# mtumalan/VisionTransformer

Measured on AMD Instinct MI355X. Metric: images/sec (512×512) ViT-B/16 seg, 1/2/4/8 MI355X + mask argmax match, higher is better.
Workload: dtype f32

## Files before the change

visiontransformer_amd/csrc/attention_bf16.hip:

```cpp
#include <type_traits>

#include "kernels.hpp"

namespace vitseg {
namespace {

constexpr int HD = 64;
constexpr int QB = 128;
constexpr int KB = 64;
constexpr float LOG2E = 1.4426950408889634f;
typedef short s16x4 __attribute__((ext_vector_type(4)));
typedef float f32x2 __attribute__((ext_vector_type(2)));

__device__ __forceinline__ int kappa(int s, int h) { return (s & 3) + 8 * (s >> 2) + 4 * h; }

template <bool DROP, bool RAGGED, bool MW, typename H>
__global__ __launch_bounds__(256, 3) void attn_bf16_kernel(const bf16_t* __restrict__ qkv, bf16_t* __restrict__ ctx,
                                                           float* __restrict__ lse, int B, int Np, int A,
                                                           DropArgs dr, const unsigned* __restrict__ maskw) {
    static_assert(!MW || (DROP && !RAGGED), "mask words: dropout on, whole 128-query blocks");
    __shared__ __attribute__((aligned(16))) bf16_t lds[2][2][KB * HD];

    const int tid = threadIdx.x, lane = tid & 63, wave = tid >> 6;
    const int li = lane & 31, lh = lane >> 5;
    const AttnTile at = attn_tile((Np + QB - 1) / QB, A);
    const int head = at.head, b = at.b;
    const int D = A * HD, ld = 3 * D;
    const size_t row0 = (size_t)b * Np;
    const size_t cls_row = (size_t)B * Np + b;
    const bf16_t* qbase = qkv + head * HD;
    const bf16_t* kbase = qkv + D + head * HD;
    const bf16_t* vbase = qkv + 2 * D + head * HD;
    const float c = 0.125f * LOG2E;

    const int q_local = at.rt * QB + wave * 32 + li;
    const bool q_valid = !RAGGED || q_local < Np;
    const size_t q_row = row0 + (q_valid ? q_local : Np - 1);
    f32x4 qf[4];
#pragma unroll
    for (int s = 0; s < 4; ++s) qf[s] = *(const f32x4*)(qbase + q_row * ld + 16 * s + 8 * lh);

    const unsigned dkey = drop_key(dr.seed, dr.stream, (unsigned)((b * A + head) * (Np + 1) + q_local));
    float m_run, l_run;
    f32x16 o[2];
    {
        float part = 0.f;
#pragma unroll
        for (int s = 0; s < 4; ++s) {
            const f32x4 kc = *(const f32x4*)(kbase + cls_row * ld + 16 * s + 8 * lh);
#pragma unroll
            for (int e = 0; e < 4; ++e) {
                const unsigned qu = __float_as_uint(qf[s][e]), ku = __float_as_uint(kc[e]);
                part = fmaf(H16<H>::lo(qu), H16<H>::lo(ku), part);
                part = fmaf(H16<H>::hi(qu), H16<H>::hi(ku), part);
            }
        }
        m_run = part + __shfl_xor(part, 32, 64);
        l_run = lh == 0 ? 1.f : 0.f;
// ... 21 lines not shown
    {
        const unsigned long long base = (unsigned long long)(kbase + row0 * ld);
        kv_rsrc[0] = (int)(unsigned)base;
        kv_rsrc[1] = (int)(unsigned)((base >> 32) & 0xffffu);
        kv_rsrc[2] = Np * ld * 2;
        kv_rsrc[3] = 0x00020000;
    }
    const int drow = 16 * __builtin_amdgcn_readfirstlane(wave) + (lane >> 3);
    unsigned voff_k[2], voff_v[2];
#pragma unroll
    for (int pc = 0; pc < 2; ++pc) {
        const int key = drow + 8 * pc;
        voff_k[pc] = (unsigned)(key * ld * 2 + (((lane & 7) ^ ((key >> 1) & 7)) << 4));
        voff_v[pc] = (unsigned)(key * ld * 2 + D * 2 + (((lane & 7) ^ (((key >> 1) & 1) << 2)) << 4));
    }
    const unsigned lds_base = (unsigned)(size_t)(__attribute__((address_space(3))) char*)&lds[0][0][0];
    auto stage = [&](int kt, int buf) {
        const unsigned soff = (unsigned)(kt * KB * ld * 2);
        const unsigned dst = lds_base + (unsigned)(buf * 2 * KB * HD * 2) + (unsigned)(__builtin_amdgcn_readfirstlane(wave) * 2048);
#pragma unroll
        for (int pc = 0; pc < 2; ++pc) {
            asm volatile("s_mov_b32 m0, %0\n\ts_nop 0\n\tbuffer_load_dwordx4 %1, %2, %3 offen lds"
                         :: "s"(dst + pc * 1024), "v"(voff_k[pc]), "s"(kv_rsrc), "s"(soff) : "memory");
            asm volatile("s_mov_b32 m0, %0\n\ts_nop 0\n\tbuffer_load_dwordx4 %1, %2, %3 offen lds"
                         :: "s"(dst + KB * HD * 2 + pc * 1024), "v"(voff_v[pc]), "s"(kv_rsrc), "s"(soff) : "memory");
        }
    };
    const int k_off = li * HD;
    const int k_sw = (li >> 1) & 7;
    const int g = lane & 15, grp = lane >> 4, tq = g >> 2, tp = g & 3;
    const int v_row = 4 * (grp >> 1) + tq;
    const int v_sw = ((tq >> 1) & 1) << 2;
    const int v_dchunk = 2 * (grp & 1) + (tp >> 1), v_half = (tp & 1) * 4;

    const int nkt = (Np + KB - 1) / KB;
    const unsigned long* mrow = nullptr;
    if (MW) {
        const int nb = Np >> 5, qg = at.rt * 4 + __builtin_amdgcn_readfirstlane(wave);
        mrow = (const unsigned long*)maskw + ((size_t)((b * A + head) * nb + qg) * nb) * 16;
    }
    TileMasks lm;
    if (MW) lm.load(mrow);
    stage(0, 0);
    asm volatile("s_waitcnt vmcnt(0)" ::: "memory");
    __syncthreads();
    constexpr float PSUM_LIMIT = sizeof(H) == 2 && std::is_same<H, f16_t>::value ? 4096.f : 65536.f;
    for (int kt = 0; kt < nkt; ++kt) {
        const int buf = kt & 1;
        if (MW) lm.wait();
        const bf16_t* Ks = lds[buf][0];
        const bf16_t* Vs = lds[buf][1];

        f32x16 st[2];
        auto scores = [&]() {
#pragma unroll
            for (int kb = 0; kb < 2; ++kb) {
#pragma unroll
                for (int r = 0; r < 16; ++r) st[kb][r] = 0.f;
#pragma unroll
                for (int s = 0; s < 4; ++s) {
                    const f32x4 kf = *(const f32x4*)&Ks[kb * 32 * HD + k_off + (((2 * s + lh) ^ k_sw) << 3)];
                    st[kb] = H16<H>::mfma(__builtin_bit_cast(bf16x8, kf), __builtin_bit_cast(bf16x8, qf[s]), st[kb]);
                }
            }
            if (RAGGED) {
#pragma unroll
                for (int kb = 0; kb < 2; ++kb)
#pragma unroll
                    for (int r = 0; r < 16; ++r)
                        if (kt * KB + kb * 32 + kappa(r, lh) >= Np) st[kb][r] = -INFINITY;
            }
        };
        scores();
        stage(min(kt + 1, nkt - 1), buf ^ 1);
        float nmc = -m_run * c;
        float psum;
        unsigned pk[2][8];
        auto exponentiate = [&]() {
            float ps0 = 0.f, ps1 = 0.f;
#pragma unroll
            for (int kb = 0; kb < 2; ++kb)
#pragma unroll
                for (int r = 0; r < 16; r += 2) {
                    float p0 = __builtin_amdgcn_exp2f(fmaf(st[kb][r], c, nmc));
                    float p1 = __builtin_amdgcn_exp2f(fmaf(st[kb][r + 1], c, nmc));
                    ps0 += p0;
                    ps1 += p1;
                    if (MW) {
                        p0 = mask_select(lm.reg(kb, r), p0);
                        p1 = mask_select(lm.reg(kb, r + 1), p1);
                    } else if (DROP) {
                        const unsigned k0 = (unsigned)(kt * KB + kb * 32);
                        p0 = drop_keep(dkey, k0 + kappa(r, lh), dr.thresh) ? p0 * dr.scale : 0.f;
                        p1 = drop_keep(dkey, k0 + kappa(r + 1, lh), dr.thresh) ? p1 * dr.scale : 0.f;
                    }
                    pk[kb][r >> 1] = H16<H>::pack2(p0, p1);
                    asm volatile("" : "+v"(pk[kb][r >> 1]));
                }
            psum = ps0 + ps1;
        };
        exponentiate();
        if (__builtin_amdgcn_ballot_w64(!(psum <= PSUM_LIMIT)) != 0) {
            scores();
            float mx = fmaxf(st[0][0], st[1][0]);
#pragma unroll
            for (int r = 1; r < 16; r += 1) mx = fmaxf(fmaxf(mx, st[0][r]), st[1][r]);
            mx = fmaxf(mx, __shfl_xor(mx, 32, 64));
            const float delta = fmaxf(mx - m_run, 0.f);
            const float alpha = __builtin_amdgcn_exp2f(-delta * c);
            l_run *= alpha;
#pragma unroll
            for (int dt = 0; dt < 2; ++dt)
#pragma unroll
                for (int r = 0; r < 16; ++r) o[dt][r] *= alpha;
            m_run += delta;
            nmc = -m_run * c;
            exponentiate();
        }
        l_run += psum;

#pragma unroll
        for (int kb = 0; kb < 2; ++kb)
#pragma unroll
            for (int s = 0; s < 2; ++s) {
                const bf16x8 pf = __builtin_bit_cast(
                    bf16x8, (uint4){pk[kb][4 * s], pk[kb][4 * s + 1], pk[kb][4 * s + 2], pk[kb][4 * s + 3]});
#pragma unroll
                for (int dt = 0; dt < 2; ++dt) {
                    const int row_a = kb * 32 + 16 * s + v_row;
                    const int ch = (4 * dt + v_dchunk) ^ v_sw;
                    const s16x4 lo = __builtin_amdgcn_ds_read_tr16_b64_v4i16(
                        (__attribute__((address_space(3))) s16x4*)(Vs + row_a * HD + (ch << 3) + v_half));
                    const s16x4 hi = __builtin_amdgcn_ds_read_tr16_b64_v4i16(
                        (__attribute__((address_space(3))) s16x4*)(Vs + (row_a + 8) * HD + (ch << 3) + v_half));
                    const bf16x8 vf = {lo[0], lo[1], lo[2], lo[3], hi[0], hi[1], hi[2], hi[3]};
                    o[dt] = H16<H>::mfma(vf, pf, o[dt]);
                }
            }

        if (MW) lm.load(mrow + (size_t)min(kt + 1, nkt - 1) * 32);
        asm volatile("s_waitcnt vmcnt(0)" ::: "memory");
        __syncthreads();
    }
    if (MW) lm.wait();

    const float l_tot = l_run + __shfl_xor(l_run, 32, 64);
    const float inv = (MW ? dr.scale : 1.0f) / l_tot;
    if (lse && q_valid && lh == 0)
        lse[((size_t)b * A + head) * (Np + 1) + q_local] = m_run * c + __builtin_amdgcn_logf(l_tot);
    if (q_valid) {
        bf16_t* out = ctx + q_row * (size_t)D + head * HD;
#pragma unroll
        for (int dt = 0; dt < 2; ++dt)
#pragma unroll
            for (int g4 = 0; g4 < 4; ++g4) {
                uint2 t;
                t.x = H16<H>::pack2(o[dt][4 * g4] * inv, o[dt][4 * g4 + 1] * inv);
                t.y = H16<H>::pack2(o[dt][4 * g4 + 2] * inv, o[dt][4 * g4 + 3] * inv);
                *(uint2*)(out + dt * 32 + 8 * g4 + 4 * lh) = t;
            }
    }
}

template <typename H>
__global__ __launch_bounds__(1024) void attn_cls_bf16_kernel(const bf16_t* __restrict__ qkv, bf16_t* __restrict__ ctx,
                                                            float* __restrict__ lse, int B, int Np, int A,
                                                            DropArgs dr) {
    extern __shared__ __attribute__((aligned(16))) float sm[];
    const int N = Np + 1;
    float* sc = sm;
    float* red = sm + ((N + 63) & ~63);
    const int tid = threadIdx.x, lane = tid & 63, wave = tid >> 6;
    const int head = blockIdx.x, b = blockIdx.y;
    const int D = A * HD, ld = 3 * D;
    const size_t row0 = (size_t)b * Np, cls_row = (size_t)B * Np + b;
    const bf16_t* qp = qkv + cls_row * ld + head * HD;
    const bf16_t* kbase = qkv + D + head * HD;
    const bf16_t* vbase = qkv + 2 * D + head * HD;
    const int sub = lane & 15, grp = lane >> 4;

    const uint2 qu = *(const uint2*)(qp + 4 * sub);
    const float qs = 0.125f * LOG2E;
    const float q0 = H16<H>::lo(qu.x) * qs, q1 = H16<H>::hi(qu.x) * qs, q2 = H16<H>::lo(qu.y) * qs, q3 = H16<H>::hi(qu.y) * qs;
    for (int base = wave * 4; base < N; base += 256) {
        float part[4];
#pragma unroll
        for (int u = 0; u < 4; ++u) {
            const int key = base + 64 * u + grp;
            part[u] = 0.f;
            if (key < N) {
                const size_t row = key < Np ? row0 + key : cls_row;
                const uint2 ku = *(const uint2*)(kbase + row * ld + 4 * sub);
                part[u] = q0 * H16<H>::lo(ku.x) + q1 * H16<H>::hi(ku.x) + q2 * H16<H>::lo(ku.y) + q3 * H16<H>::hi(ku.y);
            }
        }
#pragma unroll
        for (int u = 0; u < 4; ++u) {
            float pu = part[u];
            pu = row16_sum(pu);
            const int key = base + 64 * u + grp;
            if (sub == 0 && key < N) sc[key] = pu;
        }
    }
    __syncthreads();
    float mx = -INFINITY;
    for (int i = tid; i < N; i += 1024) mx = fmaxf(mx, sc[i]);
    mx = wave_max(mx);
    if (lane == 0) red[wave] = mx;
    __syncthreads();
    mx = red[0];
    for (int w = 1; w < 16; ++w) mx = fmaxf(mx, red[w]);
    __syncthreads();
    float sum = 0.f;
    for (int i = tid; i < N; i += 1024) {
        const float pv = __builtin_amdgcn_exp2f(sc[i] - mx);
        sc[i] = pv;
        sum += pv;
    }
    sum = wave_sum(sum);
    if (lane == 0) red[wave] = sum;
    __syncthreads();
    float ltot = 0.f;
    for (int w = 0; w < 16; ++w) ltot += red[w];
    const float inv = 1.0f / ltot;
    if (lse && tid == 0) lse[((size_t)b * A + head) * N + Np] = mx + __builtin_amdgcn_logf(ltot);
    __syncthreads();
    const int kg = tid >> 4;
    f32x4 acc = {0.f, 0.f, 0.f, 0.f};
    for (int key0 = kg; key0 < N; key0 += 256) {
        uint2 vu[4];
        float pv[4];
#pragma unroll
        for (int u = 0; u < 4; ++u) {
            const int key = min(key0 + 64 * u, N - 1);
            const size_t row = key < Np ? row0 + key : cls_row;
            vu[u] = *(const uint2*)(vbase + row * ld + 4 * sub);
            pv[u] = key0 + 64 * u < N ? sc[key] : 0.f;
            if (dr.thresh)
                pv[u] = drop_keep(drop_key(dr.seed, dr.stream, (unsigned)((b * A + head) * N + Np)), (unsigned)key,
                                  dr.thresh) ? pv[u] * dr.scale : 0.f;
        }
#pragma unroll
        for (int u = 0; u < 4; ++u) {
            acc[0] = fmaf(pv[u], H16<H>::lo(vu[u].x), acc[0]);
            acc[1] = fmaf(pv[u], H16<H>::hi(vu[u].x), acc[1]);
            acc[2] = fmaf(pv[u], H16<H>::lo(vu[u].y), acc[2]);
            acc[3] = fmaf(pv[u], H16<H>::hi(vu[u].y), acc[3]);
        }
    }
    *(f32x4*)&red[kg * 64 + 4 * sub] = acc;
    __syncthreads();
    if (tid < 64) {
        float s = 0.f;
        for (int gI = 0; gI < 64; ++gI) s += red[gI * 64 + tid];
        ctx[cls_row * (size_t)D + head * HD + tid] = H16<H>::bits(s * inv);
    }
}

}

template <typename H>
static int launch_attention_h16(const void* qkv, void* ctx, float* lse, int B, int Np, int A, DropArgs dr, hipStream_t s,
                                const unsigned* maskw) {
    VITSEG_CHECK_ARG(qkv && ctx && B > 0 && Np > 0 && A > 0, VITSEG_EINVAL, "attention_bf16: bad arguments");
    const dim3 grid((unsigned)((Np + QB - 1) / QB) * A * B);
    const bool ragged = Np % QB != 0, drop = dr.thresh != 0;
#define VITSEG_ATTN_LAUNCH(DR, RG, MWORDS)                                                                           \
    hipLaunchKernelGGL((attn_bf16_kernel<DR, RG, MWORDS, H>), grid, dim3(256), 0, s, (const bf16_t*)qkv, (bf16_t*)ctx, \
                       lse, B, Np, A, dr, maskw)
    if (drop) {
        if (ragged) VITSEG_ATTN_LAUNCH(true, true, false);
        else if (maskw) VITSEG_ATTN_LAUNCH(true, false, true);
        else VITSEG_ATTN_LAUNCH(true, false, false);
    } else {
        if (ragged) VITSEG_ATTN_LAUNCH(false, true, false); else VITSEG_ATTN_LAUNCH(false, false, false);
    }
#undef VITSEG_ATTN_LAUNCH
    VITSEG_LAUNCH_CHECK("attn_bf16");
    const size_t smem = (size_t)(((Np + 1 + 63) & ~63) + 64 * 64) * sizeof(float);
    VITSEG_CHECK_ARG(smem <= 64 * 1024, VITSEG_ESHAPE, "attention_bf16: sequence too long for the CLS kernel");
    hipLaunchKernelGGL(attn_cls_bf16_kernel<H>, dim3(A, B), dim3(1024), smem, s, (const bf16_t*)qkv, (bf16_t*)ctx, lse, B,
                       Np, A, dr);
    VITSEG_LAUNCH_CHECK("attn_cls_bf16");
    return VITSEG_OK;
}

int launch_attention_bf16(const void* qkv, void* ctx, float* lse, int B, int Np, int A, DropArgs dr, hipStream_t s,
                          bool f16, const unsigned* maskw) {
    return f16 ? launch_attention_h16<f16_t>(qkv, ctx, lse, B, Np, A, dr, s, maskw)
               : launch_attention_h16<bf16_t>(qkv, ctx, lse, B, Np, A, dr, s, maskw);
}

}
```

visiontransformer_amd/csrc/attention_f32.hip:

```cpp
#include "kernels.hpp"

namespace vitseg {
namespace {

constexpr int HD = 64;
constexpr int QB = 128;
constexpr int KB = 64;
constexpr float LOG2E = 1.4426950408889634f;

__device__ __forceinline__ int kappa(int s, int h) { return (s & 3) + 8 * (s >> 2) + 4 * h; }

template <bool RAGGED>
__global__ __launch_bounds__(256, 2) void attn_f32_kernel(const float* __restrict__ qkv, float* __restrict__ ctx,
                                                          float* __restrict__ lse, int B, int Np, int A,
                                                          DropArgs dr) {
    __shared__ __attribute__((aligned(16))) float lds[2][2][KB * HD];

    const int tid = threadIdx.x, lane = tid & 63, wave = tid >> 6;
    const int li = lane & 31, lh = lane >> 5;
    const AttnTile at = attn_tile((Np + QB - 1) / QB, A);
    const int head = at.head, b = at.b;
    const int D = A * HD, ld = 3 * D;
    const size_t row0 = (size_t)b * Np;
    const size_t cls_row = (size_t)B * Np + b;
// ... 245 lines not shown
#pragma unroll
            for (int g4 = 0; g4 < 4; ++g4) {
                f32x4 t;
#pragma unroll
                for (int e = 0; e < 4; ++e) t[e] = o[dt][4 * g4 + e] * inv;
                *(f32x4*)(out + dt * 32 + 8 * g4 + 4 * lh) = t;
            }
    }
    if (cls_blk) {
        float* red = &lds[0][0][0];
        *(f32x4*)&red[cks * 64 + 4 * cq] = co;
        if (cq == 0) {
            red[1024 + cks] = cm;
            red[1040 + cks] = cl;
        }
        __syncthreads();
        if (tid < 64) {
            float M = red[1024];
#pragma unroll
            for (int g = 1; g < 16; ++g) M = fmaxf(M, red[1024 + g]);
            float L = 0.f, O = 0.f;
#pragma unroll
            for (int g = 0; g < 16; ++g) {
                const float w = __builtin_amdgcn_exp2f(red[1024 + g] - M);
                L = fmaf(red[1040 + g], w, L);
                O = fmaf(red[g * 64 + tid], w, O);
            }
            ctx[cls_row * (size_t)D + head * HD + tid] = O / L;
            if (lse && tid == 0) lse[((size_t)b * A + head) * (Np + 1) + Np] = M + __builtin_amdgcn_logf(L);
        }
    }
}

__global__ __launch_bounds__(1024) void attn_cls_f32_kernel(const float* __restrict__ qkv, float* __restrict__ ctx,
                                                           float* __restrict__ lse, int B, int Np, int A,
                                                           DropArgs dr) {
    extern __shared__ __attribute__((aligned(16))) float sm[];
    const int N = Np + 1;
    float* sc = sm;
    float* red = sm + ((N + 63) & ~63);
    const int tid = threadIdx.x, lane = tid & 63, wave = tid >> 6;
    const int head = blockIdx.x, b = blockIdx.y;
    const int D = A * HD, ld = 3 * D;
    const size_t row0 = (size_t)b * Np, cls_row = (size_t)B * Np + b;
    const float* qp = qkv + cls_row * ld + head * HD;
    const float* kbase = qkv + D + head * HD;
    const float* vbase = qkv + 2 * D + head * HD;
    const int sub = lane & 15, grp = lane >> 4;

    f32x4 q4 = *(const f32x4*)(qp + 4 * sub);
    const float qs = 0.125f * LOG2E;
    for (int e = 0; e < 4; ++e) q4[e] *= qs;
    for (int base = wave * 4; base < N; base += 256) {
        float part[4];
#pragma unroll
        for (int u = 0; u < 4; ++u) {
            const int key = base + 64 * u + grp;
            part[u] = 0.f;
            if (key < N) {
                const size_t row = key < Np ? row0 + key : cls_row;
                const f32x4 k4 = *(const f32x4*)(kbase + row * ld + 4 * sub);
                part[u] = q4[0] * k4[0] + q4[1] * k4[1] + q4[2] * k4[2] + q4[3] * k4[3];
            }
        }
#pragma unroll
        for (int u = 0; u < 4; ++u) {
            float pu = part[u];
            pu = row16_sum(pu);
            const int key = base + 64 * u + grp;
            if (sub == 0 && key < N) sc[key] = pu;
        }
    }
    __syncthreads();
    float mx = -INFINITY;
    for (int i = tid; i < N; i += 1024) mx = fmaxf(mx, sc[i]);
    mx = wave_max(mx);
    if (lane == 0) red[wave] = mx;
    __syncthreads();
    mx = red[0];
    for (int w = 1; w < 16; ++w) mx = fmaxf(mx, red[w]);
    __syncthreads();
    float sum = 0.f;
    for (int i = tid; i < N; i += 1024) {
        const float pv = __builtin_amdgcn_exp2f(sc[i] - mx);
        sc[i] = pv;
        sum += pv;
    }
    sum = wave_sum(sum);
    if (lane == 0) red[wave] = sum;
    __syncthreads();
    float ltot = 0.f;
    for (int w = 0; w < 16; ++w) ltot += red[w];
    const float inv = 1.0f / ltot;
    if (lse && tid == 0) lse[((size_t)b * A + head) * N + Np] = mx + __builtin_amdgcn_logf(ltot);
    __syncthreads();
    const int kg = tid >> 4;
    f32x4 acc = {0.f, 0.f, 0.f, 0.f};
    for (int key0 = kg; key0 < N; key0 += 256) {
        f32x4 v4[4];
        float pv[4];
#pragma unroll
        for (int u = 0; u < 4; ++u) {
            const int key = min(key0 + 64 * u, N - 1);
            const size_t row = key < Np ? row0 + key : cls_row;
            v4[u] = *(const f32x4*)(vbase + row * ld + 4 * sub);
            pv[u] = key0 + 64 * u < N ? sc[key] : 0.f;
            if (dr.thresh)
                pv[u] = drop_keep(drop_key(dr.seed, dr.stream, (unsigned)((b * A + head) * N + Np)), (unsigned)key,
                                  dr.thresh) ? pv[u] * dr.scale : 0.f;
        }
#pragma unroll
        for (int u = 0; u < 4; ++u)
            for (int e = 0; e < 4; ++e) acc[e] = fmaf(pv[u], v4[u][e], acc[e]);
    }
    *(f32x4*)&red[kg * 64 + 4 * sub] = acc;
    __syncthreads();
    if (tid < 64) {
        float s = 0.f;
        for (int g = 0; g < 64; ++g) s += red[g * 64 + tid];
        ctx[cls_row * (size_t)D + head * HD + tid] = s * inv;
    }
}

}

int launch_attention_f32(const float* qkv, float* ctx, float* lse, int B, int Np, int A, DropArgs dr, hipStream_t s,
                         bool x3) {
    VITSEG_CHECK_ARG(qkv && ctx && B > 0 && Np > 0 && A > 0, VITSEG_EINVAL, "attention_f32: bad arguments");
    const dim3 grid((unsigned)((Np + QB - 1) / QB) * A * B);
    if (x3) {
        VITSEG_CHECK_ARG(!lse && !dr.thresh, VITSEG_EINVAL, "attention (x3) is an inference path: no lse / dropout");
        if (int rc = launch_attention_x3_main(qkv, ctx, B, Np, A, s)) return rc;
    } else if (Np % QB == 0) {
        hipLaunchKernelGGL(attn_f32_kernel<false>, grid, dim3(256), 0, s, qkv, ctx, lse, B, Np, A, dr);
    } else {
        hipLaunchKernelGGL(attn_f32_kernel<true>, grid, dim3(256), 0, s, qkv, ctx, lse, B, Np, A, dr);
    }
    VITSEG_LAUNCH_CHECK("attn_f32");
    if (!x3) return VITSEG_OK;
    const size_t smem = (size_t)(((Np + 1 + 63) & ~63) + 64 * 64) * sizeof(float);
    VITSEG_CHECK_ARG(smem <= 64 * 1024, VITSEG_ESHAPE, "attention_f32: sequence too long for the CLS kernel");
    hipLaunchKernelGGL(attn_cls_f32_kernel, dim3(A, B), dim3(1024), smem, s, qkv, ctx, lse, B, Np, A, dr);
    VITSEG_LAUNCH_CHECK("attn_cls_f32");
    return VITSEG_OK;
}

}
```

visiontransformer_amd/csrc/attention_x3.hip:

```cpp
#include "kernels.hpp"

namespace vitseg {
namespace {

constexpr int HD = 64;
constexpr int QB = 128;
constexpr int KB = 64;
constexpr float LOG2E = 1.4426950408889634f;
constexpr float LO_SCALE = 2048.f, LO_INV = 1.0f / 2048.f;
typedef short s16x4 __attribute__((ext_vector_type(4)));

__device__ __forceinline__ int kappa(int s, int h) { return (s & 3) + 8 * (s >> 2) + 4 * h; }

__device__ __forceinline__ void split8(const f32x4& a, const f32x4& b, f32x4& hi, f32x4& lo) {
    unsigned h[4], l[4];
#pragma unroll
    for (int j = 0; j < 2; ++j) {
        const _Float16 a0 = (_Float16)a[2 * j], a1 = (_Float16)a[2 * j + 1];
        const _Float16 b0 = (_Float16)b[2 * j], b1 = (_Float16)b[2 * j + 1];
        h[j] = __builtin_bit_cast(unsigned, f16x2{a0, a1});
        h[2 + j] = __builtin_bit_cast(unsigned, f16x2{b0, b1});
        l[j] = H16<f16_t>::pack2((a[2 * j] - (float)a0) * LO_SCALE, (a[2 * j + 1] - (float)a1) * LO_SCALE);
        l[2 + j] = H16<f16_t>::pack2((b[2 * j] - (float)b0) * LO_SCALE, (b[2 * j + 1] - (float)b1) * LO_SCALE);
    }
    hi = __builtin_bit_cast(f32x4, (uint4){h[0], h[1], h[2], h[3]});
    lo = __builtin_bit_cast(f32x4, (uint4){l[0], l[1], l[2], l[3]});
}

template <bool RAGGED>
__global__ __launch_bounds__(256, 2) void attn_x3_kernel(const float* __restrict__ qkv, float* __restrict__ ctx, int B, int Np,
                                                         int A) {
    __shared__ __attribute__((aligned(16))) unsigned short lds[2][2][2][KB * HD];

    const int tid = threadIdx.x, lane = tid & 63, wave = tid >> 6;
    const int li = lane & 31, lh = lane >> 5;
    const AttnTile at = attn_tile((Np + QB - 1) / QB, A);
    const int head = at.head, b = at.b;
    const int D = A * HD, ld = 3 * D;
    const size_t row0 = (size_t)b * Np;
    const size_t cls_row = (size_t)B * Np + b;
    const float* qbase = qkv + head * HD;
    const float* kbase = qkv + D + head * HD;
    const float* vbase = qkv + 2 * D + head * HD;
    const float c = 0.125f * LOG2E;

    const int q_local = at.rt * QB + wave * 32 + li;
    const bool q_valid = q_local < Np;
    const size_t q_row = row0 + (q_valid ? q_local : Np - 1);
    f32x4 qh[4], ql[4];
    float m_run, l_run;
    f32x16 o0[2], o1[2];
    {
        float part = 0.f;
#pragma unroll
        for (int s = 0; s < 4; ++s) {
            const float* qp = qbase + q_row * ld + 16 * s + 8 * lh;
            const float* kp = kbase + cls_row * ld + 16 * s + 8 * lh;
            const f32x4 qa = *(const f32x4*)qp, qb = *(const f32x4*)(qp + 4);
            const f32x4 ka = *(const f32x4*)kp, kb = *(const f32x4*)(kp + 4);
#pragma unroll
            for (int e = 0; e < 4; ++e) part = fmaf(qb[e], kb[e], fmaf(qa[e], ka[e], part));
            split8(qa, qb, qh[s], ql[s]);
        }
        m_run = part + __shfl_xor(part, 32, 64);
        l_run = lh == 0 ? 1.f : 0.f;
#pragma unroll
        for (int dt = 0; dt < 2; ++dt)
#pragma unroll
            for (int g4 = 0; g4 < 4; ++g4) {
// ... 11 lines not shown
    auto gload = [&](int kt) {
#pragma unroll
        for (int i = 0; i < 2; ++i) {
            int key = kt * KB + lr + 32 * i;
            if (RAGGED) key = min(key, Np - 1);
            const size_t off = (row0 + key) * ld + 8 * lc;
            rk[i][0] = *(const f32x4*)(kbase + off);
            rk[i][1] = *(const f32x4*)(kbase + off + 4);
            rv[i][0] = *(const f32x4*)(vbase + off);
            rv[i][1] = *(const f32x4*)(vbase + off + 4);
        }
    };
    auto swrite = [&](int buf) {
#pragma unroll
        for (int i = 0; i < 2; ++i) {
            const int key = lr + 32 * i;
            f32x4 hi, lo;
            split8(rk[i][0], rk[i][1], hi, lo);
            const int kpos = key * HD + ((lc ^ ((key >> 1) & 7)) << 3);
            *(f32x4*)&lds[buf][0][0][kpos] = hi;
            *(f32x4*)&lds[buf][0][1][kpos] = lo;
            split8(rv[i][0], rv[i][1], hi, lo);
            const int vpos = key * HD + ((lc ^ (((key >> 1) & 1) << 2)) << 3);
            *(f32x4*)&lds[buf][1][0][vpos] = hi;
            *(f32x4*)&lds[buf][1][1][vpos] = lo;
        }
    };
    const int k_off = li * HD;
    const int k_sw = (li >> 1) & 7;
    const int g = lane & 15, grp = lane >> 4, tq = g >> 2, tp = g & 3;
    const int v_row = 4 * (grp >> 1) + tq;
    const int v_sw = ((tq >> 1) & 1) << 2;
    const int v_dchunk = 2 * (grp & 1) + (tp >> 1), v_half = (tp & 1) * 4;

    const int nkt = (Np + KB - 1) / KB;
    gload(0);
    swrite(0);
    __syncthreads();
    for (int kt = 0; kt < nkt; ++kt) {
        const int buf = kt & 1;
        gload(min(kt + 1, nkt - 1));
        __builtin_amdgcn_sched_barrier(0);
        const unsigned short* Kh = lds[buf][0][0];
        const unsigned short* Kl = lds[buf][0][1];
        const unsigned short* Vh = lds[buf][1][0];
        const unsigned short* Vl = lds[buf][1][1];

        f32x16 st[2];
#pragma unroll
        for (int kb = 0; kb < 2; ++kb) {
            f32x16 s1;
#pragma unroll
            for (int r = 0; r < 16; ++r) st[kb][r] = s1[r] = 0.f;
#pragma unroll
            for (int s = 0; s < 4; ++s) {
                const int pos = kb * 32 * HD + k_off + (((2 * s + lh) ^ k_sw) << 3);
                const bf16x8 kh = __builtin_bit_cast(bf16x8, *(const f32x4*)&Kh[pos]);
                const bf16x8 kl = __builtin_bit_cast(bf16x8, *(const f32x4*)&Kl[pos]);
                st[kb] = H16<f16_t>::mfma(kh, __builtin_bit_cast(bf16x8, qh[s]), st[kb]);
                s1 = H16<f16_t>::mfma(kl, __builtin_bit_cast(bf16x8, qh[s]), s1);
                s1 = H16<f16_t>::mfma(kh, __builtin_bit_cast(bf16x8, ql[s]), s1);
            }
#pragma unroll
            for (int r = 0; r < 16; ++r) st[kb][r] = fmaf(s1[r], LO_INV, st[kb][r]);
        }
        if (RAGGED) {
#pragma unroll
            for (int kb = 0; kb < 2; ++kb)
#pragma unroll
                for (int r = 0; r < 16; ++r)
                    if (kt * KB + kb * 32 + kappa(r, lh) >= Np) st[kb][r] = -INFINITY;
        }
        float mx = fmaxf(st[0][0], st[1][0]);
#pragma unroll
        for (int r = 1; r < 16; r += 1) mx = fmaxf(fmaxf(mx, st[0][r]), st[1][r]);
        mx = fmaxf(mx, __shfl_xor(mx, 32, 64));
        const float m_new = fmaxf(m_run, mx);
        if (__builtin_amdgcn_ballot_w64(m_new > m_run) != 0) {
            const float alpha = __builtin_amdgcn_exp2f((m_run - m_new) * c);
// ... 36 lines not shown
                    const int row_a = kb * 32 + 16 * s + v_row;
                    const int ch = (4 * dt + v_dchunk) ^ v_sw;
                    const int p0 = row_a * HD + (ch << 3) + v_half, p8 = (row_a + 8) * HD + (ch << 3) + v_half;
                    const s16x4 hlo = __builtin_amdgcn_ds_read_tr16_b64_v4i16((__attribute__((address_space(3))) s16x4*)(Vh + p0));
                    const s16x4 hhi = __builtin_amdgcn_ds_read_tr16_b64_v4i16((__attribute__((address_space(3))) s16x4*)(Vh + p8));
                    const s16x4 llo = __builtin_amdgcn_ds_read_tr16_b64_v4i16((__attribute__((address_space(3))) s16x4*)(Vl + p0));
                    const s16x4 lhi = __builtin_amdgcn_ds_read_tr16_b64_v4i16((__attribute__((address_space(3))) s16x4*)(Vl + p8));
                    const bf16x8 vh = {hlo[0], hlo[1], hlo[2], hlo[3], hhi[0], hhi[1], hhi[2], hhi[3]};
                    const bf16x8 vl = {llo[0], llo[1], llo[2], llo[3], lhi[0], lhi[1], lhi[2], lhi[3]};
                    o0[dt] = H16<f16_t>::mfma(vh, pfh, o0[dt]);
                    o1[dt] = H16<f16_t>::mfma(vl, pfh, o1[dt]);
                    o1[dt] = H16<f16_t>::mfma(vh, pfl, o1[dt]);
                }
            }

        swrite(buf ^ 1);
        __syncthreads();
    }

    const float l_tot = l_run + __shfl_xor(l_run, 32, 64);
    const float inv = 1.0f / l_tot;
    if (q_valid) {
        float* out = ctx + q_row * (size_t)D + head * HD;
#pragma unroll
        for (int dt = 0; dt < 2; ++dt)
#pragma unroll
            for (int g4 = 0; g4 < 4; ++g4) {
                f32x4 t;
#pragma unroll
                for (int e = 0; e < 4; ++e) t[e] = fmaf(o1[dt][4 * g4 + e], LO_INV, o0[dt][4 * g4 + e]) * inv;
                *(f32x4*)(out + dt * 32 + 8 * g4 + 4 * lh) = t;
            }
    }
}

}

int launch_attention_x3_main(const float* qkv, float* ctx, int B, int Np, int A, hipStream_t s) {
    const dim3 grid((unsigned)((Np + QB - 1) / QB) * A * B);
    if (Np % QB == 0)
        hipLaunchKernelGGL(attn_x3_kernel<false>, grid, dim3(256), 0, s, qkv, ctx, B, Np, A);
    else
        hipLaunchKernelGGL(attn_x3_kernel<true>, grid, dim3(256), 0, s, qkv, ctx, B, Np, A);
    VITSEG_LAUNCH_CHECK("attn_x3");
    return VITSEG_OK;
}

}
```

visiontransformer_amd/csrc/common.hpp:

```cpp
#pragma once
#include <hip/hip_runtime.h>
#include <stdint.h>

#include "../../include/vitseg.h"

namespace vitseg {

constexpr int WAVE = 64;

typedef float f32x4 __attribute__((ext_vector_type(4)));
typedef float f32x16 __attribute__((ext_vector_type(16)));
typedef short bf16x8 __attribute__((ext_vector_type(8)));
typedef short bf16x4 __attribute__((ext_vector_type(4)));

void set_error(const char* fmt, ...);
int hip_fail(hipError_t e, const char* what);

enum Opt {
    OPT_NO_F32P = 0,
    OPT_NO_P8,
    OPT_NO_H16P,
    OPT_NO_RAGGED_P8,
    OPT_NO_DROPMASK,
    OPT_DROPW_LIMIT_MB,
// ... 15 lines not shown
        if (!(cond)) {                    \
            ::vitseg::set_error(__VA_ARGS__); \
            return (code);                \
        }                                 \
    } while (0)

#define VITSEG_LAUNCH_CHECK(what)                               \
    do {                                                        \
        hipError_t e__ = hipGetLastError();                     \
        if (e__ != hipSuccess) return ::vitseg::hip_fail(e__, what); \
    } while (0)

inline size_t up256(size_t v) { return (v + 255) & ~(size_t)255; }

__device__ __forceinline__ int xcd_remap(int bid, int nwg) {
    const int q = nwg >> 3, r = nwg & 7, xcd = bid & 7, idx = bid >> 3;
    const int base = (xcd < r) ? xcd * (q + 1) : r * (q + 1) + (xcd - r) * q;
    return base + idx;
}

struct AttnTile {
    int rt, head, b;
};
__device__ __forceinline__ AttnTile attn_tile(int ntiles, int A) {
    const int t = xcd_remap(blockIdx.x, gridDim.x);
    const int bh = t / ntiles;
    AttnTile r;
    r.rt = t - bh * ntiles;
    r.b = bh / A;
    r.head = bh - r.b * A;
    return r;
}

__host__ __device__ __forceinline__ unsigned fmix32(unsigned h) {
    h ^= h >> 16;
    h *= 0x85ebca6bu;
    h ^= h >> 13;
    h *= 0xc2b2ae35u;
    h ^= h >> 16;
    return h;
}
__host__ __device__ __forceinline__ unsigned drop_key(unsigned seed, unsigned stream, unsigned major) {
    return fmix32(seed ^ (stream * 0x9E3779B1u) ^ (major * 0x85EBCA77u));
}
__host__ __device__ __forceinline__ unsigned mad24(unsigned a, unsigned k, unsigned c) {
#if defined(__HIP_DEVICE_COMPILE__)
    return __umul24(a, k) + c;
#else
    return (unsigned)(((unsigned long long)(a & 0xffffffu) * (k & 0xffffffu) + c) & 0xffffffffull);
#endif
}
__host__ __device__ __forceinline__ unsigned drop_pair_hash(unsigned key, unsigned pair) {
    unsigned h = mad24(pair, 0x9E3779u, key);
    h ^= h >> 15;
    h *= 0x85EBCA6Bu;
    return h;
}
__host__ __device__ __forceinline__ bool drop_keep(unsigned key, unsigned minor, unsigned thresh) {
    const unsigned h = drop_pair_hash(key, minor >> 1);
    return ((minor & 1u) ? (h >> 16) : (h & 0xffffu)) >= thresh;
}
struct DropArgs {
    unsigned thresh;
    unsigned seed;
    unsigned stream;
    float scale;
// ... 4 lines not shown
        d.thresh = (unsigned)((double)p * 65536.0 + 0.5);
        if (d.thresh == 0) d.thresh = 1;
        d.seed = seed;
        d.stream = stream;
        d.scale = 1.0f / (1.0f - p);
    }
    return d;
}

inline size_t attn_dropmask_words(int B, int Np, int A) { return (size_t)B * A * (Np / 32) * Np; }
typedef unsigned long u64x8 __attribute__((ext_vector_type(8)));
struct TileMasks {
    u64x8 v[4];
    __device__ __forceinline__ void load(const unsigned long* p) {
#if defined(__HIP_DEVICE_COMPILE__)
        asm volatile(
            "s_load_dwordx16 %0, %4, 0x0\n\ts_load_dwordx16 %1, %4, 0x40\n\t"
            "s_load_dwordx16 %2, %4, 0x80\n\ts_load_dwordx16 %3, %4, 0xc0"
            : "=&s"(v[0]), "=&s"(v[1]), "=&s"(v[2]), "=&s"(v[3])
            : "s"(p));
#endif
    }
    __device__ __forceinline__ void wait() {
#if defined(__HIP_DEVICE_COMPILE__)
        asm volatile("s_waitcnt lgkmcnt(0)" : "+s"(v[0]), "+s"(v[1]), "+s"(v[2]), "+s"(v[3]));
#endif
    }
    __device__ __forceinline__ unsigned long reg(int kb, int r) const { return v[2 * kb + (r >> 3)][r & 7]; }
};
__device__ __forceinline__ float mask_select(unsigned long lanes, float v) {
#if defined(__HIP_DEVICE_COMPILE__)
    float o;
    asm("v_cndmask_b32 %0, 0, %1, %2" : "=v"(o) : "v"(v), "s"(lanes));
    return o;
#else
    return v;
#endif
}

#if defined(__HIP_DEVICE_COMPILE__)
#define VITSEG_DPP(x, ctrl, rmask) \
    __builtin_bit_cast(float, __builtin_amdgcn_update_dpp(0, __builtin_bit_cast(int, (x)), (ctrl), (rmask), 0xf, false))
__device__ __forceinline__ float wave_sum(float v) {
    v += VITSEG_DPP(v, 0xb1, 0xf);
    v += VITSEG_DPP(v, 0x4e, 0xf);
    v += VITSEG_DPP(v, 0x141, 0xf);
    v += VITSEG_DPP(v, 0x140, 0xf);
    v += VITSEG_DPP(v, 0x142, 0xa);
    v += VITSEG_DPP(v, 0x143, 0xc);
    return __builtin_bit_cast(float, __builtin_amdgcn_readlane(__builtin_bit_cast(int, v), 63));
}
__device__ __forceinline__ float row16_sum(float v) {
    v += VITSEG_DPP(v, 0xb1, 0xf);
    v += VITSEG_DPP(v, 0x4e, 0xf);
    v += VITSEG_DPP(v, 0x141, 0xf);
    v += VITSEG_DPP(v, 0x140, 0xf);
    return v;
}
__device__ __forceinline__ float wave_max(float v) {
#define VITSEG_DPP_KEEP(x, ctrl, rmask) \
    __builtin_bit_cast(float, __builtin_amdgcn_update_dpp(__builtin_bit_cast(int, (x)), __builtin_bit_cast(int, (x)), (ctrl), (rmask), 0xf, false))
    v = fmaxf(v, VITSEG_DPP_KEEP(v, 0xb1, 0xf));
    v = fmaxf(v, VITSEG_DPP_KEEP(v, 0x4e, 0xf));
    v = fmaxf(v, VITSEG_DPP_KEEP(v, 0x141, 0xf));
    v = fmaxf(v, VITSEG_DPP_KEEP(v, 0x140, 0xf));
    v = fmaxf(v, VITSEG_DPP_KEEP(v, 0x142, 0xa));
// ... 120 lines not shown
```

Measured before the change: 616.5.

## Fuse CLS-token attention into main attention kernel with heavy-first tile scheduling

```diff
diff --git a/visiontransformer_amd/csrc/attention_bf16.hip b/visiontransformer_amd/csrc/attention_bf16.hip
--- a/visiontransformer_amd/csrc/attention_bf16.hip
+++ b/visiontransformer_amd/csrc/attention_bf16.hip
@@ -23,7 +23,7 @@
 
     const int tid = threadIdx.x, lane = tid & 63, wave = tid >> 6;
     const int li = lane & 31, lh = lane >> 5;
-    const AttnTile at = attn_tile((Np + QB - 1) / QB, A);
+    const AttnTile at = attn_tile_heavy_first((Np + QB - 1) / QB, A);
     const int head = at.head, b = at.b;
     const int D = A * HD, ld = 3 * D;
     const size_t row0 = (size_t)b * Np;
@@ -111,6 +111,103 @@
     const int v_row = 4 * (grp >> 1) + tq;
     const int v_sw = ((tq >> 1) & 1) << 2;
     const int v_dchunk = 2 * (grp & 1) + (tp >> 1), v_half = (tp & 1) * 4;
+
+    constexpr bool CLS_LDS = DROP && !MW;
+    __shared__ __attribute__((aligned(16))) float cls_st[CLS_LDS ? 4 * 256 * 4 : 4];
+    const bool cls_blk = at.rt == 0;
+    const int cq = tid & 7, cks = tid >> 3;
+    const int ckr = (cks & 25) | ((cks & 2) << 1) | ((cks & 4) >> 1);
+    const int ck_pos = ckr * HD + ((cq ^ ((ckr >> 1) & 7)) << 3);
+    const int cv_pos = ckr * HD + ((cq ^ (((ckr >> 1) & 1) << 2)) << 3);
+    uint4 cqp = {0u, 0u, 0u, 0u};
+    float co[8] = {0.f, 0.f, 0.f, 0.f, 0.f, 0.f, 0.f, 0.f};
+    float cm = -1e30f, cl = 0.f;
+    unsigned ckey = 0;
+    auto sum8 = [](float t) {
+        t += __builtin_bit_cast(float, __builtin_amdgcn_update_dpp(0, __builtin_bit_cast(int, t), 0xb1, 0xf, 0xf, true));
+        t += __builtin_bit_cast(float, __builtin_amdgcn_update_dpp(0, __builtin_bit_cast(int, t), 0x4e, 0xf, 0xf, true));
+        t += __builtin_bit_cast(float, __builtin_amdgcn_update_dpp(0, __builtin_bit_cast(int, t), 0x141, 0xf, 0xf, true));
+        return t;
+    };
+    auto unpack8 = [](const uint4& u, float (&f)[8]) {
+        f[0] = H16<H>::lo(u.x); f[1] = H16<H>::hi(u.x); f[2] = H16<H>::lo(u.y); f[3] = H16<H>::hi(u.y);
+        f[4] = H16<H>::lo(u.z); f[5] = H16<H>::hi(u.z); f[6] = H16<H>::lo(u.w); f[7] = H16<H>::hi(u.w);
+    };
+    auto cls_score = [&](const float (&q8)[8], const uint4& ku) {
+        float k8[8];
+        unpack8(ku, k8);
+        float t = 0.f;
+#pragma unroll
+        for (int e = 0; e < 8; ++e) t = fmaf(q8[e], k8[e], t);
+        return sum8(t) * c;
+    };
+    auto st_load = [&]() {
+#pragma unroll
+        for (int j = 0; j < 2; ++j) {
+            const f32x4 t = *(const f32x4*)&cls_st[(j * 256 + tid) * 4];
+#pragma unroll
+            for (int e = 0; e < 4; ++e) co[4 * j + e] = t[e];
+        }
+        const f32x2 ml = *(const f32x2*)&cls_st[(2 * 256 + tid) * 4];
+        cm = ml[0];
+        cl = ml[1];
+        cqp = *(const uint4*)&cls_st[(3 * 256 + tid) * 4];
+    };
+    auto st_store = [&]() {
+#pragma unroll
+        for (int j = 0; j < 2; ++j)
+            *(f32x4*)&cls_st[(j * 256 + tid) * 4] = f32x4{co[4 * j], co[4 * j + 1], co[4 * j + 2], co[4 * j + 3]};
+        *(f32x2*)&cls_st[(2 * 256 + tid) * 4] = f32x2{cm, cl};
+    };
+    if (cls_blk) {
+        cqp = *(const uint4*)(qbase + cls_row * ld + 8 * cq);
+        if (DROP) ckey = drop_key(dr.seed, dr.stream, (unsigned)((b * A + head) * (Np + 1) + Np));
+        float q8[8];
+        unpack8(cqp, q8);
+        const float scc = cls_score(q8, *(const uint4*)(kbase + cls_row * ld + 8 * cq));
+        if (cks == 0) {
+            cm = scc;
+            cl = 1.f;
+            unpack8(*(const uint4*)(vbase + cls_row * ld + 8 * cq), co);
+            if (DROP && !drop_keep(ckey, (unsigned)Np, dr.thresh)) {
+#pragma unroll
+                for (int e = 0; e < 8; ++e) co[e] = 0.f;
+            }
+        }
+        if (CLS_LDS) {
+            st_store();
+            *(uint4*)&cls_st[(3 * 256 + tid) * 4] = cqp;
+        }
+    }
+    auto cls_tile = [&](int kt, const bf16_t* Ks, const bf16_t* Vs) {
+        float q8[8], sc[2];
+        if (CLS_LDS) st_load();
+        unpack8(cqp, q8);
+        uint4 vu[2];
+#pragma unroll
+        for (int u = 0; u < 2; ++u) {
+            sc[u] = cls_score(q8, *(const uint4*)&Ks[u * 32 * HD + ck_pos]);
+            vu[u] = *(const uint4*)&Vs[u * 32 * HD + cv_pos];
+            if (RAGGED && kt * KB + ckr + 32 * u >= Np) sc[u] = -INFINITY;
+        }
+        const float m_new = fmaxf(fmaxf(cm, sc[0]), sc[1]);
+        const float alpha = __builtin_amdgcn_exp2f(cm - m_new);
+        cm = m_new;
+        cl *= alpha;
+#pragma unroll
+        for (int e = 0; e < 8; ++e) co[e] *= alpha;
+#pragma unroll
+        for (int u = 0; u < 2; ++u) {
+            float pv = __builtin_amdgcn_exp2f(sc[u] - m_new);
+            cl += pv;
+            if (DROP && !drop_keep(ckey, (unsigned)(kt * KB + ckr + 32 * u), dr.thresh)) pv = 0.f;
+            float v8[8];
+            unpack8(vu[u], v8);
+#pragma unroll
+            for (int e = 0; e < 8; ++e) co[e] = fmaf(pv, v8[e], co[e]);
+        }
+        if (CLS_LDS) st_store();
+    };
 
     const int nkt = (Np + KB - 1) / KB;
     const unsigned long* mrow = nullptr;
@@ -166,8 +263,8 @@
                     ps0 += p0;
                     ps1 += p1;
                     if (MW) {
-                        p0 = mask_select(lm.reg(kb, r), p0);
-                        p1 = mask_select(lm.reg(kb, r + 1), p1);
+                        p0 = mask_select(lm.reg(kb, r), p0, ps0);
+                        p1 = mask_select(lm.reg(kb, r + 1), p1, ps1);
                     } else if (DROP) {
                         const unsigned k0 = (unsigned)(kt * KB + kb * 32);
                         p0 = drop_keep(dkey, k0 + kappa(r, lh), dr.thresh) ? p0 * dr.scale : 0.f;
@@ -217,6 +314,7 @@
                 }
             }
 
+        if (cls_blk) cls_tile(kt, Ks, Vs);
         if (MW) lm.load(mrow + (size_t)min(kt + 1, nkt - 1) * 32);
         asm volatile("s_waitcnt vmcnt(0)" ::: "memory");
         __syncthreads();
@@ -239,100 +337,30 @@
                 *(uint2*)(out + dt * 32 + 8 * g4 + 4 * lh) = t;
             }
     }
-}
-
-template <typename H>
-__global__ __launch_bounds__(1024) void attn_cls_bf16_kernel(const bf16_t* __restrict__ qkv, bf16_t* __restrict__ ctx,
-                                                            float* __restrict__ lse, int B, int Np, int A,
-                                                            DropArgs dr) {
-    extern __shared__ __attribute__((aligned(16))) float sm[];
-    const int N = Np + 1;
-    float* sc = sm;
-    float* red = sm + ((N + 63) & ~63);
-    const int tid = threadIdx.x, lane = tid & 63, wave = tid >> 6;
-    const int head = blockIdx.x, b = blockIdx.y;
-    const int D = A * HD, ld = 3 * D;
-    const size_t row0 = (size_t)b * Np, cls_row = (size_t)B * Np + b;
-    const bf16_t* qp = qkv + cls_row * ld + head * HD;
-    const bf16_t* kbase = qkv + D + head * HD;
-    const bf16_t* vbase = qkv + 2 * D + head * HD;
-    const int sub = lane & 15, grp = lane >> 4;
-
-    const uint2 qu = *(const uint2*)(qp + 4 * sub);
-    const float qs = 0.125f * LOG2E;
-    const float q0 = H16<H>::lo(qu.x) * qs, q1 = H16<H>::hi(qu.x) * qs, q2 = H16<H>::lo(qu.y) * qs, q3 = H16<H>::hi(qu.y) * qs;
-    for (int base = wave * 4; base < N; base += 256) {
-        float part[4];
-#pragma unroll
-        for (int u = 0; u < 4; ++u) {
-            const int key = base + 64 * u + grp;
-            part[u] = 0.f;
-            if (key < N) {
-                const size_t row = key < Np ? row0 + key : cls_row;
-                const uint2 ku = *(const uint2*)(kbase + row * ld + 4 * sub);
-                part[u] = q0 * H16<H>::lo(ku.x) + q1 * H16<H>::hi(ku.x) + q2 * H16<H>::lo(ku.y) + q3 * H16<H>::hi(ku.y);
-            }
-        }
-#pragma unroll
-        for (int u = 0; u < 4; ++u) {
-            float pu = part[u];
-            pu = row16_sum(pu);
-            const int key = base + 64 * u + grp;
-            if (sub == 0 && key < N) sc[key] = pu;
-        }
-    }
-    __syncthreads();
-    float mx = -INFINITY;
-    for (int i = tid; i < N; i += 1024) mx = fmaxf(mx, sc[i]);
-    mx = wave_max(mx);
-    if (lane == 0) red[wave] = mx;
-    __syncthreads();
-    mx = red[0];
-    for (int w = 1; w < 16; ++w) mx = fmaxf(mx, red[w]);
-    __syncthreads();
-    float sum = 0.f;
-    for (int i = tid; i < N; i += 1024) {
-        const float pv = __builtin_amdgcn_exp2f(sc[i] - mx);
-        sc[i] = pv;
-        sum += pv;
-    }
-    sum = wave_sum(sum);
-    if (lane == 0) red[wave] = sum;
-    __syncthreads();
-    float ltot = 0.f;
-    for (int w = 0; w < 16; ++w) ltot += red[w];
-    const float inv = 1.0f / ltot;
-    if (lse && tid == 0) lse[((size_t)b * A + head) * N + Np] = mx + __builtin_amdgcn_logf(ltot);
-    __syncthreads();
-    const int kg = tid >> 4;
-    f32x4 acc = {0.f, 0.f, 0.f, 0.f};
-    for (int key0 = kg; key0 < N; key0 += 256) {
-        uint2 vu[4];
-        float pv[4];
-#pragma unroll
-        for (int u = 0; u < 4; ++u) {
-            const int key = min(key0 + 64 * u, N - 1);
-            const size_t row = key < Np ? row0 + key : cls_row;
-            vu[u] = *(const uint2*)(vbase + row * ld + 4 * sub);
-            pv[u] = key0 + 64 * u < N ? sc[key] : 0.f;
-            if (dr.thresh)
-                pv[u] = drop_keep(drop_key(dr.seed, dr.stream, (unsigned)((b * A + head) * N + Np)), (unsigned)key,
-                                  dr.thresh) ? pv[u] * dr.scale : 0.f;
-        }
-#pragma unroll
-        for (int u = 0; u < 4; ++u) {
-            acc[0] = fmaf(pv[u], H16<H>::lo(vu[u].x), acc[0]);
-            acc[1] = fmaf(pv[u], H16<H>::hi(vu[u].x), acc[1]);
-            acc[2] = fmaf(pv[u], H16<H>::lo(vu[u].y), acc[2]);
-            acc[3] = fmaf(pv[u], H16<H>::hi(vu[u].y), acc[3]);
-        }
-    }
-    *(f32x4*)&red[kg * 64 + 4 * sub] = acc;
-    __syncthreads();
-    if (tid < 64) {
-        float s = 0.f;
-        for (int gI = 0; gI < 64; ++gI) s += red[gI * 64 + tid];
-        ctx[cls_row * (size_t)D + head * HD + tid] = H16<H>::bits(s * inv);
+    if (cls_blk) {
+        float* red = (float*)&lds[0][0][0];
+        if (CLS_LDS) st_load();
+#pragma unroll
+        for (int e = 0; e < 8; e += 4) *(f32x4*)&red[cks * 64 + 8 * cq + e] = f32x4{co[e], co[e + 1], co[e + 2], co[e + 3]};
+        if (cq == 0) {
+            red[2048 + cks] = cm;
+            red[2080 + cks] = cl;
+        }
+        __syncthreads();
+        if (tid < 64) {
+            float M = red[2048];
+#pragma unroll
+            for (int gI = 1; gI < 32; ++gI) M = fmaxf(M, red[2048 + gI]);
+            float L = 0.f, O = 0.f;
+#pragma unroll 8
+            for (int gI = 0; gI < 32; ++gI) {
+                const float w = __builtin_amdgcn_exp2f(red[2048 + gI] - M);
+                L = fmaf(red[2080 + gI], w, L);
+                O = fmaf(red[gI * 64 + tid], w, O);
+            }
+            ctx[cls_row * (size_t)D + head * HD + tid] = H16<H>::bits(O * ((DROP ? dr.scale : 1.0f) / L));
+            if (lse && tid == 0) lse[((size_t)b * A + head) * (Np + 1) + Np] = M + __builtin_amdgcn_logf(L);
+        }
     }
 }
 
@@ -356,11 +384,6 @@
     }
 #undef VITSEG_ATTN_LAUNCH
     VITSEG_LAUNCH_CHECK("attn_bf16");
-    const size_t smem = (size_t)(((Np + 1 + 63) & ~63) + 64 * 64) * sizeof(float);
-    VITSEG_CHECK_ARG(smem <= 64 * 1024, VITSEG_ESHAPE, "attention_bf16: sequence too long for the CLS kernel");
-    hipLaunchKernelGGL(attn_cls_bf16_kernel<H>, dim3(A, B), dim3(1024), smem, s, (const bf16_t*)qkv, (bf16_t*)ctx, lse, B,
-                       Np, A, dr);
-    VITSEG_LAUNCH_CHECK("attn_cls_bf16");
     return VITSEG_OK;
 }
 
diff --git a/visiontransformer_amd/csrc/attention_f32.hip b/visiontransformer_amd/csrc/attention_f32.hip
--- a/visiontransformer_amd/csrc/attention_f32.hip
+++ b/visiontransformer_amd/csrc/attention_f32.hip
@@ -301,96 +301,6 @@
     }
 }
 
-__global__ __launch_bounds__(1024) void attn_cls_f32_kernel(const float* __restrict__ qkv, float* __restrict__ ctx,
-                                                           float* __restrict__ lse, int B, int Np, int A,
-                                                           DropArgs dr) {
-    extern __shared__ __attribute__((aligned(16))) float sm[];
-    const int N = Np + 1;
-    float* sc = sm;
-    float* red = sm + ((N + 63) & ~63);
-    const int tid = threadIdx.x, lane = tid & 63, wave = tid >> 6;
-    const int head = blockIdx.x, b = blockIdx.y;
-    const int D = A * HD, ld = 3 * D;
-    const size_t row0 = (size_t)b * Np, cls_row = (size_t)B * Np + b;
-    const float* qp = qkv + cls_row * ld + head * HD;
-    const float* kbase = qkv + D + head * HD;
-    const float* vbase = qkv + 2 * D + head * HD;
-    const int sub = lane & 15, grp = lane >> 4;
-
-    f32x4 q4 = *(const f32x4*)(qp + 4 * sub);
-    const float qs = 0.125f * LOG2E;
-    for (int e = 0; e < 4; ++e) q4[e] *= qs;
-    for (int base = wave * 4; base < N; base += 256) {
-        float part[4];
-#pragma unroll
-        for (int u = 0; u < 4; ++u) {
-            const int key = base + 64 * u + grp;
-            part[u] = 0.f;
-            if (key < N) {
-                const size_t row = key < Np ? row0 + key : cls_row;
-                const f32x4 k4 = *(const f32x4*)(kbase + row * ld + 4 * sub);
-                part[u] = q4[0] * k4[0] + q4[1] * k4[1] + q4[2] * k4[2] + q4[3] * k4[3];
-            }
-        }
-#pragma unroll
-        for (int u = 0; u < 4; ++u) {
-            float pu = part[u];
-            pu = row16_sum(pu);
-            const int key = base + 64 * u + grp;
-            if (sub == 0 && key < N) sc[key] = pu;
-        }
-    }
-    __syncthreads();
-    float mx = -INFINITY;
-    for (int i = tid; i < N; i += 1024) mx = fmaxf(mx, sc[i]);
-    mx = wave_max(mx);
-    if (lane == 0) red[wave] = mx;
-    __syncthreads();
-    mx = red[0];
-    for (int w = 1; w < 16; ++w) mx = fmaxf(mx, red[w]);
-    __syncthreads();
-    float sum = 0.f;
-    for (int i = tid; i < N; i += 1024) {
-        const float pv = __builtin_amdgcn_exp2f(sc[i] - mx);
-        sc[i] = pv;
-        sum += pv;
-    }
-    sum = wave_sum(sum);
-    if (lane == 0) red[wave] = sum;
-    __syncthreads();
-    float ltot = 0.f;
-    for (int w = 0; w < 16; ++w) ltot += red[w];
-    const float inv = 1.0f / ltot;
-    if (lse && tid == 0) lse[((size_t)b * A + head) * N + Np] = mx + __builtin_amdgcn_logf(ltot);
-    __syncthreads();
-    const int kg = tid >> 4;
-    f32x4 acc = {0.f, 0.f, 0.f, 0.f};
-    for (int key0 = kg; key0 < N; key0 += 256) {
-        f32x4 v4[4];
-        float pv[4];
-#pragma unroll
-        for (int u = 0; u < 4; ++u) {
-            const int key = min(key0 + 64 * u, N - 1);
-            const size_t row = key < Np ? row0 + key : cls_row;
-            v4[u] = *(const f32x4*)(vbase + row * ld + 4 * sub);
-            pv[u] = key0 + 64 * u < N ? sc[key] : 0.f;
-            if (dr.thresh)
-                pv[u] = drop_keep(drop_key(dr.seed, dr.stream, (unsigned)((b * A + head) * N + Np)), (unsigned)key,
-                                  dr.thresh) ? pv[u] * dr.scale : 0.f;
-        }
-#pragma unroll
-        for (int u = 0; u < 4; ++u)
-            for (int e = 0; e < 4; ++e) acc[e] = fmaf(pv[u], v4[u][e], acc[e]);
-    }
-    *(f32x4*)&red[kg * 64 + 4 * sub] = acc;
-    __syncthreads();
-    if (tid < 64) {
-        float s = 0.f;
-        for (int g = 0; g < 64; ++g) s += red[g * 64 + tid];
-        ctx[cls_row * (size_t)D + head * HD + tid] = s * inv;
-    }
-}
-
 }
 
 int launch_attention_f32(const float* qkv, float* ctx, float* lse, int B, int Np, int A, DropArgs dr, hipStream_t s,
@@ -399,18 +309,14 @@
     const dim3 grid((unsigned)((Np + QB - 1) / QB) * A * B);
     if (x3) {
         VITSEG_CHECK_ARG(!lse && !dr.thresh, VITSEG_EINVAL, "attention (x3) is an inference path: no lse / dropout");
-        if (int rc = launch_attention_x3_main(qkv, ctx, B, Np, A, s)) return rc;
-    } else if (Np % QB == 0) {
+        return launch_attention_x3_main(qkv, ctx, B, Np, A, s);
+    }
+    if (Np % QB == 0) {
         hipLaunchKernelGGL(attn_f32_kernel<false>, grid, dim3(256), 0, s, qkv, ctx, lse, B, Np, A, dr);
     } else {
         hipLaunchKernelGGL(attn_f32_kernel<true>, grid, dim3(256), 0, s, qkv, ctx, lse, B, Np, A, dr);
     }
     VITSEG_LAUNCH_CHECK("attn_f32");
-    if (!x3) return VITSEG_OK;
-    const size_t smem = (size_t)(((Np + 1 + 63) & ~63) + 64 * 64) * sizeof(float);
-    VITSEG_CHECK_ARG(smem <= 64 * 1024, VITSEG_ESHAPE, "attention_f32: sequence too long for the CLS kernel");
-    hipLaunchKernelGGL(attn_cls_f32_kernel, dim3(A, B), dim3(1024), smem, s, qkv, ctx, lse, B, Np, A, dr);
-    VITSEG_LAUNCH_CHECK("attn_cls_f32");
     return VITSEG_OK;
 }
 
diff --git a/visiontransformer_amd/csrc/attention_x3.hip b/visiontransformer_amd/csrc/attention_x3.hip
--- a/visiontransformer_amd/csrc/attention_x3.hip
+++ b/visiontransformer_amd/csrc/attention_x3.hip
@@ -34,7 +34,7 @@
 
     const int tid = threadIdx.x, lane = tid & 63, wave = tid >> 6;
     const int li = lane & 31, lh = lane >> 5;
-    const AttnTile at = attn_tile((Np + QB - 1) / QB, A);
+    const AttnTile at = attn_tile_heavy_first((Np + QB - 1) / QB, A);
     const int head = at.head, b = at.b;
     const int D = A * HD, ld = 3 * D;
     const size_t row0 = (size_t)b * Np;
@@ -112,6 +112,84 @@
     const int v_row = 4 * (grp >> 1) + tq;
     const int v_sw = ((tq >> 1) & 1) << 2;
     const int v_dchunk = 2 * (grp & 1) + (tp >> 1), v_half = (tp & 1) * 4;
+
+    const bool cls_blk = at.rt == 0;
+    const int cq = tid & 7, cks = tid >> 3;
+    const int ckr = (cks & 25) | ((cks & 2) << 1) | ((cks & 4) >> 1);
+    const int ck_pos = ckr * HD + ((cq ^ ((ckr >> 1) & 7)) << 3);
+    const int cv_pos = ckr * HD + ((cq ^ (((ckr >> 1) & 1) << 2)) << 3);
+    float cq8[8] = {0.f, 0.f, 0.f, 0.f, 0.f, 0.f, 0.f, 0.f};
+    float co0[8] = {0.f, 0.f, 0.f, 0.f, 0.f, 0.f, 0.f, 0.f}, co1[8] = {0.f, 0.f, 0.f, 0.f, 0.f, 0.f, 0.f, 0.f};
+    float cm = -1e30f, cl = 0.f;
+    auto sum8 = [](float t) {
+        t += __builtin_bit_cast(float, __builtin_amdgcn_update_dpp(0, __builtin_bit_cast(int, t), 0xb1, 0xf, 0xf, true));
+        t += __builtin_bit_cast(float, __builtin_amdgcn_update_dpp(0, __builtin_bit_cast(int, t), 0x4e, 0xf, 0xf, true));
+        t += __builtin_bit_cast(float, __builtin_amdgcn_update_dpp(0, __builtin_bit_cast(int, t), 0x141, 0xf, 0xf, true));
+        return t;
+    };
+    auto halves8 = [](const unsigned short* p, float (&f)[8]) {
+        const f16x8 h = *(const f16x8*)p;
+#pragma unroll
+        for (int e = 0; e < 8; ++e) f[e] = (float)h[e];
+    };
+    if (cls_blk) {
+        const float* qp = qbase + cls_row * ld + 8 * cq;
+        const float* kp = kbase + cls_row * ld + 8 * cq;
+        float t = 0.f;
+#pragma unroll
+        for (int e = 0; e < 8; ++e) {
+            cq8[e] = qp[e] * c;
+            t = fmaf(cq8[e], kp[e], t);
+        }
+        const float scc = sum8(t);
+        if (cks == 0) {
+            cm = scc;
+            cl = 1.f;
+            const float* vp = vbase + cls_row * ld + 8 * cq;
+#pragma unroll
+            for (int e = 0; e < 8; ++e) co0[e] = vp[e];
+        }
+    }
+    auto cls_tile = [&](int kt, const unsigned short* Kh, const unsigned short* Kl, const unsigned short* Vh,
+                        const unsigned short* Vl) {
+        float sc[2];
+#pragma unroll
+        for (int u = 0; u < 2; ++u) {
+            float kh8[8], kl8[8];
+            halves8(Kh + u * 32 * HD + ck_pos, kh8);
+            halves8(Kl + u * 32 * HD + ck_pos, kl8);
+            float t0 = 0.f, t1 = 0.f;
+#pragma unroll
+            for (int e = 0; e < 8; ++e) {
+                t0 = fmaf(cq8[e], kh8[e], t0);
+                t1 = fmaf(cq8[e], kl8[e], t1);
+            }
+            sc[u] = sum8(fmaf(t1, LO_INV, t0));
+            if (RAGGED && kt * KB + ckr + 32 * u >= Np) sc[u] = -INFINITY;
+        }
+        const float m_new = fmaxf(fmaxf(cm, sc[0]), sc[1]);
+        const float alpha = __builtin_amdgcn_exp2f(cm - m_new);
+        cm = m_new;
+        cl *= alpha;
+#pragma unroll
+        for (int e = 0; e < 8; ++e) {
+            co0[e] *= alpha;
+            co1[e] *= alpha;
+        }
+#pragma unroll
+        for (int u = 0; u < 2; ++u) {
+            const float pv = __builtin_amdgcn_exp2f(sc[u] - m_new);
+            cl += pv;
+            float vh8[8], vl8[8];
+            halves8(Vh + u * 32 * HD + cv_pos, vh8);
+            halves8(Vl + u * 32 * HD + cv_pos, vl8);
+#pragma unroll
+            for (int e = 0; e < 8; ++e) {
+                co0[e] = fmaf(pv, vh8[e], co0[e]);
+                co1[e] = fmaf(pv, vl8[e], co1[e]);
+            }
+        }
+    };
 
     const int nkt = (Np + KB - 1) / KB;
     gload(0);
@@ -125,6 +203,7 @@
         const unsigned short* Kl = lds[buf][0][1];
         const unsigned short* Vh = lds[buf][1][0];
         const unsigned short* Vl = lds[buf][1][1];
+        if (cls_blk) cls_tile(kt, Kh, Kl, Vh, Vl);
 
         f32x16 st[2];
 #pragma unroll
@@ -227,6 +306,34 @@
                 *(f32x4*)(out + dt * 32 + 8 * g4 + 4 * lh) = t;
             }
     }
+    if (cls_blk) {
+        float* red = (float*)&lds[0][0][0][0];
+#pragma unroll
+        for (int e = 0; e < 8; e += 4) {
+            f32x4 t;
+#pragma unroll
+            for (int j = 0; j < 4; ++j) t[j] = fmaf(co1[e + j], LO_INV, co0[e + j]);
+            *(f32x4*)&red[cks * 64 + 8 * cq + e] = t;
+        }
+        if (cq == 0) {
+            red[2048 + cks] = cm;
+            red[2080 + cks] = cl;
+        }
+        __syncthreads();
+        if (tid < 64) {
+            float M = red[2048];
+#pragma unroll
+            for (int gI = 1; gI < 32; ++gI) M = fmaxf(M, red[2048 + gI]);
+            float L = 0.f, O = 0.f;
+#pragma unroll 8
+            for (int gI = 0; gI < 32; ++gI) {
+                const float w = __builtin_amdgcn_exp2f(red[2048 + gI] - M);
+                L = fmaf(red[2080 + gI], w, L);
+                O = fmaf(red[gI * 64 + tid], w, O);
+            }
+            ctx[cls_row * (size_t)D + head * HD + tid] = O / L;
+        }
+    }
 }
 
 }
diff --git a/visiontransformer_amd/csrc/common.hpp b/visiontransformer_amd/csrc/common.hpp
--- a/visiontransformer_amd/csrc/common.hpp
+++ b/visiontransformer_amd/csrc/common.hpp
@@ -71,6 +71,30 @@
     return r;
 }
 
+__device__ __forceinline__ AttnTile attn_tile_heavy_first(int ntiles, int A) {
+    const int nwg = gridDim.x, bid = blockIdx.x;
+    const int q = nwg >> 3, r = nwg & 7, xcd = bid & 7, idx = bid >> 3;
+    const int base = (xcd < r) ? xcd * (q + 1) : r * (q + 1) + (xcd - r) * q;
+    const int cnt = q + (xcd < r ? 1 : 0);
+    int t = base + idx;
+    if (ntiles > 1) {
+        const int hb = (base + ntiles - 1) / ntiles;
+        const int nh = (base + cnt + ntiles - 1) / ntiles - hb;
+        if (idx < nh) {
+            t = (hb + idx) * ntiles;
+        } else {
+            const int k = base - hb + (idx - nh);
+            t = k + k / (ntiles - 1) + 1;
+        }
+    }
+    const int bh = t / ntiles;
+    AttnTile o;
+    o.rt = t - bh * ntiles;
+    o.b = bh / A;
+    o.head = bh - o.b * A;
+    return o;
+}
+
 __host__ __device__ __forceinline__ unsigned fmix32(unsigned h) {
     h ^= h >> 16;
     h *= 0x85ebca6bu;
@@ -141,6 +165,15 @@
 #if defined(__HIP_DEVICE_COMPILE__)
     float o;
     asm("v_cndmask_b32 %0, 0, %1, %2" : "=v"(o) : "v"(v), "s"(lanes));
+    return o;
+#else
+    return v;
+#endif
+}
+__device__ __forceinline__ float mask_select(unsigned long lanes, float v, float after) {
+#if defined(__HIP_DEVICE_COMPILE__)
+    float o;
+    asm("v_cndmask_b32 %0, 0, %1, %2" : "=v"(o) : "v"(v), "s"(lanes), "v"(after));
     return o;
 #else
     return v;
```

Result: no change. 617.2, median of 6 (+0.1%).
